# eromero-vlc/superbblas

Measured on AMD Instinct MI355X. Metric: lattice contraction GFLOP/s + permute GB/s, 16^4 spin×color, 1/2/4/8 GPUs, higher is better.
Workload: dtype complex<f64>

## Files before the change

superbblas_amd/csrc/capi.cpp:

```cpp
#include "plan.h"
#include <atomic>
#include <algorithm>
#include <functional>
#include <memory>
#include <unordered_map>

#include <rccl/rccl.h>

#include <cstdlib>
#include <cstring>
#include <mutex>

namespace sbx {
BsrOp *bsr_create(int nd, int ni, int dtype, const std::vector<std::vector<Range>> &pi,
                  const Coor &dimi, const std::vector<std::vector<Range>> &pd, const Coor &dimd,
                  const Coor &blocki, const Coor &blockd, bool block_im_fast,
                  const std::vector<const int *> &ii, const std::vector<const int *> &jj,
                  const std::vector<const void *> &v, const std::vector<int> &devs, bool reverse_jj,
                  const Comm &comm, const Coor *kroni = nullptr, const Coor *krond = nullptr,
                  const std::vector<const void *> *kronv = nullptr);
void bsr_destroy(BsrOp *op);
void bsr_krylov(const BsrOp &op, const Scalar &alpha, const std::string &oi,
                const std::string &od, const DistTensor &x, const Coor &fromx, const Coor &sizex,
                const Scalar &beta, const DistTensor &y, const Coor &fromy, const Coor &sizey,
// ... 365 lines not shown
        if (live) *live = l;
    });
}

int sbx_tune_set(const char *key, long long value) {
    return guard([&] {
        if (!key) throw Error("tune_set: null key");
        const std::string k(key);
        if (k == "copy.budget") g_copy_tune.budget = (long)value;
        else if (k == "copy.run") g_copy_tune.run = (long)value;
        else if (k == "copy.nt") g_copy_tune.nt = (int)value;
        else if (k == "copy.max_elems") g_copy_tune.max_elems = (long)value;
        else if (k == "copy.pair") g_copy_tune.pair = (int)value;
        else if (k == "copy.order") g_copy_tune.order = (int)value;
        else if (k == "copy.trans") g_copy_tune.trans = (int)value;
        else if (k == "copy.btrans") g_copy_tune.btrans = (int)value;
        else if (k == "gemm.max_bytes") g_gemm_tune.max_bytes = (long)value;
        else if (k == "gemm.loaders") g_gemm_tune.loaders = (int)value;
        else if (k == "gemm.dma_spread") g_gemm_tune.dma_spread = (int)value;
        else if (k == "gemm.dma_nt") g_gemm_tune.dma_nt = (int)value;
        else if (k == "gemm.lean") g_gemm_tune.lean = (int)value;
        else if (k == "gemm.skinny") g_gemm_tune.skinny = (int)value;
        else if (k == "bsr.variant") g_bsr_tune.variant = (int)value;
        else if (k == "bsr.row_max_cols") g_bsr_tune.row_max_cols = (long)value;
        else if (k == "bsr.split_max_cols") g_bsr_tune.split_max_cols = (long)value;
        else if (k == "bsr.split_cw") g_bsr_tune.split_cw = (int)value;
        else if (k == "bsr.split_jb") g_bsr_tune.split_jb = (int)value;
        else if (k == "bsr.split_ilv") g_bsr_tune.split_ilv = (int)value;
        else if (k == "bsr.kron_mfma") g_bsr_tune.kron_mfma = (int)value;
        else if (k == "bsr.kron_mfma_min_cols") g_bsr_tune.kron_mfma_min_cols = (long)value;
        else if (k == "bsr.kron_pack") g_bsr_tune.kron_pack = (int)value;
        else if (k == "bsr.kron_xlds") g_bsr_tune.kron_xlds = (int)value;
        else if (k == "bsr.kron_ylds") g_bsr_tune.kron_ylds = (int)value;
        else if (k == "bsr.kron_spin") g_bsr_tune.kron_spin = (int)value;
        else if (k == "bsr.kron_adj") g_bsr_tune.kron_adj = (int)value;
        else if (k == "bsr.kron_spin_min_cols") g_bsr_tune.kron_spin_min_cols = (long)value;
        else if (k == "bsr.kron_order") g_bsr_tune.kron_order = (int)value;
        else if (k == "bsr.nt") g_bsr_tune.nt = (int)value;
        else if (k == "dense.wave") g_dense_wave = (int)value;
        else if (k == "bsr.blk_pd") g_bsr_tune.blk_pd = (int)value;
        else if (k == "bsr.blk_mfma") g_bsr_tune.blk_mfma = (int)value;
        else if (k == "bsr.blk_min") g_bsr_tune.blk_min = (int)value;
        else if (k == "bsr.mixed") g_bsr_tune.mixed = (int)value;
        else if (k == "bsr.adj_inplace") g_bsr_tune.adj_inplace = (int)value;
        else if (k == "bsr.adj_copy_bytes") throw Error("tune_set: bsr.adj_copy_bytes is read-only");
        else if (k == "bsr.tile") g_bsr_tune.tile = (int)value;
        else if (k == "bsr.tile_min_cols") g_bsr_tune.tile_min_cols = value;
        else if (k == "gemm.m3") g_gemm_tune.m3 = (int)value;
        else if (k == "gemm.splits") g_gemm_tune.splits = (int)value;
        else if (k == "gemm.t48") g_gemm_tune.t48 = (int)value;
        else if (k == "gemm.share_ab") g_gemm_tune.share_ab = (int)value;
        else if (k == "gemm.herm") g_gemm_tune.herm = (int)value;
        else if (k == "gemm.frag") g_gemm_tune.frag = (int)value;
        else if (k == "gemm.dot_wgs") g_gemm_tune.dot_wgs = (int)value;
        else if (k == "gemm.frag_tall") g_gemm_tune.frag_tall = (int)value;
        else if (k == "gemm.frag_pair") g_gemm_tune.frag_pair = (int)value;
        else if (k == "gemm.frag_nt") g_gemm_tune.frag_nt = (int)value;
        else if (k == "gemm.frag_small") g_gemm_tune.frag_small = (int)value;
        else if (k == "gemm.frag_uk") g_gemm_tune.frag_uk = (int)value;
        else if (k == "gemm.frag_waves") g_gemm_tune.frag_waves = (int)value;
        else if (k == "gemm.clock") {
            g_gemm_tune.clock = (int)value;
            unsigned long long v[3];
            gemm_clock_read(current_device(), v, true);
        }
        else if (k == "dist.reduce") g_dist_reduce = (int)value;
// ... 12 lines not shown
}

int sbx_tune_get(const char *key, long long *value) {
    return guard([&] {
        if (!key || !value) throw Error("tune_get: null argument");
        const std::string k(key);
        if (k == "copy.budget") *value = g_copy_tune.budget;
        else if (k == "copy.run") *value = g_copy_tune.run;
        else if (k == "copy.nt") *value = g_copy_tune.nt;
        else if (k == "copy.max_elems") *value = g_copy_tune.max_elems;
        else if (k == "copy.pair") *value = g_copy_tune.pair;
        else if (k == "copy.order") *value = g_copy_tune.order;
        else if (k == "copy.trans") *value = g_copy_tune.trans;
        else if (k == "copy.btrans") *value = g_copy_tune.btrans;
        else if (k == "copy.last_pair") *value = g_copy_tune.last_pair;
        else if (k == "gemm.max_bytes") *value = g_gemm_tune.max_bytes;
        else if (k == "gemm.loaders") *value = g_gemm_tune.loaders;
        else if (k == "gemm.dma_spread") *value = g_gemm_tune.dma_spread;
        else if (k == "gemm.dma_nt") *value = g_gemm_tune.dma_nt;
        else if (k == "gemm.lean") *value = g_gemm_tune.lean;
        else if (k == "gemm.last_lean") *value = g_gemm_tune.last_lean;
        else if (k == "gemm.skinny") *value = g_gemm_tune.skinny;
        else if (k == "bsr.variant") *value = g_bsr_tune.variant;
        else if (k == "bsr.row_max_cols") *value = g_bsr_tune.row_max_cols;
        else if (k == "bsr.split_max_cols") *value = g_bsr_tune.split_max_cols;
        else if (k == "bsr.split_cw") *value = g_bsr_tune.split_cw;
        else if (k == "bsr.split_jb") *value = g_bsr_tune.split_jb;
        else if (k == "bsr.split_ilv") *value = g_bsr_tune.split_ilv;
        else if (k == "bsr.kron_mfma") *value = g_bsr_tune.kron_mfma;
        else if (k == "bsr.kron_mfma_min_cols") *value = g_bsr_tune.kron_mfma_min_cols;
        else if (k == "bsr.kron_pack") *value = g_bsr_tune.kron_pack;
        else if (k == "bsr.kron_xlds") *value = g_bsr_tune.kron_xlds;
        else if (k == "bsr.kron_ylds") *value = g_bsr_tune.kron_ylds;
        else if (k == "bsr.kron_spin") *value = g_bsr_tune.kron_spin;
        else if (k == "bsr.kron_adj") *value = g_bsr_tune.kron_adj;
        else if (k == "bsr.kron_spin_min_cols") *value = g_bsr_tune.kron_spin_min_cols;
        else if (k == "bsr.kron_order") *value = g_bsr_tune.kron_order;
        else if (k == "bsr.nt") *value = g_bsr_tune.nt;
        else if (k == "dense.wave") *value = g_dense_wave;
        else if (k == "bsr.blk_pd") *value = g_bsr_tune.blk_pd;
        else if (k == "bsr.blk_mfma") *value = g_bsr_tune.blk_mfma;
        else if (k == "bsr.blk_min") *value = g_bsr_tune.blk_min;
        else if (k == "bsr.tile") *value = g_bsr_tune.tile;
        else if (k == "bsr.tile_min_cols") *value = g_bsr_tune.tile_min_cols;
        else if (k == "bsr.mixed") *value = g_bsr_tune.mixed;
        else if (k == "bsr.last_kernel") *value = g_bsr_tune.last;
        else if (k == "bsr.last_mixed") *value = g_bsr_tune.last_mixed;
        else if (k == "bsr.adj_inplace") *value = g_bsr_tune.adj_inplace;
        else if (k == "bsr.adj_copy_bytes") *value = g_bsr_tune.adj_copy_bytes;
        else if (k == "gemm.m3") *value = g_gemm_tune.m3;
        else if (k == "gemm.splits") *value = g_gemm_tune.splits;
        else if (k == "gemm.t48") *value = g_gemm_tune.t48;
        else if (k == "gemm.share_ab") *value = g_gemm_tune.share_ab;
        else if (k == "gemm.herm") *value = g_gemm_tune.herm;
        else if (k == "gemm.last_herm") *value = g_gemm_tune.last_herm;
        else if (k == "gemm.frag") *value = g_gemm_tune.frag;
        else if (k == "gemm.dot_wgs") *value = g_gemm_tune.dot_wgs;
        else if (k == "gemm.frag_tall") *value = g_gemm_tune.frag_tall;
        else if (k == "gemm.frag_pair") *value = g_gemm_tune.frag_pair;
        else if (k == "gemm.frag_nt") *value = g_gemm_tune.frag_nt;
        else if (k == "gemm.frag_small") *value = g_gemm_tune.frag_small;
        else if (k == "gemm.frag_uk") *value = g_gemm_tune.frag_uk;
        else if (k == "gemm.frag_waves") *value = g_gemm_tune.frag_waves;
        else if (k == "gemm.clock") *value = g_gemm_tune.clock;
        else if (k == "gemm.clock_cycles" || k == "gemm.clock_ticks" || k == "gemm.clock_launches") {
            unsigned long long v[3];
// ... 1058 lines not shown
```

superbblas_amd/csrc/kernels_bsr.hip:

```cpp
#include "elem_ops.h"
#include "sbx_internal.h"

#include <algorithm>
#include <type_traits>

namespace sbx {
BsrTune g_bsr_tune;
namespace {

struct BsrArgs {
    long block_rows;
    int bi, bd;
    const int *ii;
    const int *jj;
    const void *v;
    int block_im_fast;
    const void *x;
    long ldx;
    long x_rows;
    void *y;
    long ldy;
    long ncols;
    double alpha_re, alpha_im;
    int add;
// ... 1501 lines not shown
    }
}

template <typename E>
void gather_typed(const void *src, const int *perm, long nblocks, long be, bool cj, void *dst,
                  hipStream_t s) {
    const long blocks = std::min((nblocks * be + 255) / 256, 65536L);
    hipLaunchKernelGGL(gather_blocks_kernel<E>, dim3((unsigned)blocks), dim3(256), 0, s,
                       (const E *)src, perm, nblocks, be, cj ? 1 : 0, (E *)dst);
    SBX_HIP_CHECK(hipGetLastError());
}

}

void launch_gather_blocks(int t, const void *src, const int *perm, long nblocks, long block_elems,
                          bool conj_values, void *dst, int device) {
    if (nblocks == 0 || block_elems == 0) return;
    set_device(device);
    hipStream_t s = get_stream(device);
    switch (t) {
    case SBX_CDOUBLE: return gather_typed<double2>(src, perm, nblocks, block_elems, conj_values, dst, s);
    case SBX_CFLOAT: return gather_typed<float2>(src, perm, nblocks, block_elems, conj_values, dst, s);
    case SBX_DOUBLE: return gather_typed<double>(src, perm, nblocks, block_elems, false, dst, s);
    case SBX_FLOAT: return gather_typed<float>(src, perm, nblocks, block_elems, false, dst, s);
    case SBX_CHALF: return gather_typed<f16x2>(src, perm, nblocks, block_elems, conj_values, dst, s);
    case SBX_HALF: return gather_typed<f16>(src, perm, nblocks, block_elems, false, dst, s);
    default: throw Error("bsr: unsupported type");
    }
}

void launch_bsr(const BsrDesc &d, int device) {
    if (d.block_rows == 0 || d.ncols == 0) return;
    g_bsr_tune.last = 0;
    set_device(device);
    hipStream_t s = get_stream(device);
    BsrArgs a{};
    a.block_rows = d.block_rows;
    a.bi = d.bi;
    a.bd = d.bd;
    a.ii = d.ii;
    a.jj = d.jj;
    a.v = d.v;
    a.block_im_fast = d.block_im_fast ? 1 : 0;
    a.x = d.x;
    a.ldx = d.ldx;
    a.x_rows = d.x_rows;
    a.y = d.y;
    a.ldy = d.ldy;
    a.ncols = d.ncols;
    a.alpha_re = d.alpha.re;
    a.alpha_im = d.alpha.im;
    a.add = d.add ? 1 : 0;
    a.ilv = 2;
    a.nt = g_bsr_tune.nt;
    a.tiles[0] = d.tiles[0];
    a.tiles[1] = d.tiles[1];
    if (d.adj_ent) {
        const bool yr = d.y_row_major, xr = d.x_row_major;
        if (d.tv == SBX_CFLOAT && d.t == SBX_CDOUBLE) return launch_adj<float2, double2>(a, d.adj_ent, yr, xr, s);
        if (d.tv == SBX_FLOAT && d.t == SBX_DOUBLE) return launch_adj<float, double>(a, d.adj_ent, yr, xr, s);
        if (d.tv == SBX_CHALF && d.t == SBX_CFLOAT) return launch_adj<f16x2, float2>(a, d.adj_ent, yr, xr, s);
        if (d.tv == SBX_HALF && d.t == SBX_FLOAT) return launch_adj<f16, float>(a, d.adj_ent, yr, xr, s);
        if (d.tv != d.t) throw Error("bsr: unsupported pair of value and vector types");
        switch (d.t) {
        case SBX_CDOUBLE: return launch_adj<double2, double2>(a, d.adj_ent, yr, xr, s);
        case SBX_CFLOAT: return launch_adj<float2, float2>(a, d.adj_ent, yr, xr, s);
// ... 27 lines not shown
```

superbblas_amd/csrc/kernels_bsr_kron.hip:

```cpp
#include "elem_ops.h"
#include "sbx_internal.h"

#include <algorithm>
#include <type_traits>

namespace sbx {
namespace {

struct KronArgs {
    long block_rows;
    int nnz;
    int bi, bd, ki, kd;
    const int *jj;
    const void *v;
    const void *kron;
    int block_im_fast;
    const void *x;
    void *y;
    long ncols;
    double alpha_re, alpha_im;
    int add;
    int ylds;
    long x_rows;
    const int *perm;
// ... 196 lines not shown
    const E *__restrict__ x = (const E *)p.x;
    E *__restrict__ y = (E *)p.y;
    const long total = p.block_rows * p.bi * p.ncols * p.ki;
    for (long idx = blockIdx.x * 256L + threadIdx.x; idx < total; idx += (long)gridDim.x * 256L) {
        const int a = (int)(idx % p.ki);
        long t = idx / p.ki;
        const long c = t % p.ncols;
        t /= p.ncols;
        const int i = (int)(t % p.bi);
        const long r = t / p.bi;
        E acc = Ops<E>::zero();
        for (int mu = 0; mu < p.nnz; ++mu) {
            const long j = r * p.nnz + mu;
            const E *xs = x + (long)p.jj[j] * p.bd * p.ncols * p.kd + c * p.kd;
            const E *K = kron + (long)mu * p.ki * p.kd;
            const E *U = v + j * p.bi * p.bd;
            for (int b = 0; b < p.kd; ++b) {
                const E k = p.block_im_fast ? K[a + b * p.ki] : K[a * p.kd + b];
                if (!Ops<E>::nonzero(k)) continue;
                E s = Ops<E>::zero();
                for (int d = 0; d < p.bd; ++d) {
                    const E u = p.block_im_fast ? U[i + d * p.bi] : U[i * p.bd + d];
                    s = Ops<E>::fma(u, xs[d * p.ncols * p.kd + b], s);
                }
                acc = Ops<E>::fma(k, s, acc);
            }
        }
        E o = Ops<E>::scale(acc, p.alpha_re, p.alpha_im);
        if (p.add) o = Ops<E>::add(o, y[idx]);
        y[idx] = o;
    }
}

template <int NNZ, bool kpf = false, int XL = 0>
__global__ void __launch_bounds__(256) bsr_kron_mfma_kernel(const KronArgs p, int ngroups) {
    typedef double2 E;
    const E *__restrict__ x = (const E *)p.x;
    E *__restrict__ y = (E *)p.y;
    const int lane = threadIdx.x & 63;
    const int w = __builtin_amdgcn_readfirstlane(threadIdx.x >> 6);
    const long nchunk = (p.block_rows + 3) / 4;
    const int bid = blockIdx.x, nwg = gridDim.x;
    const int xcd = bid & 7, q8 = nwg >> 3, r8 = nwg & 7;
    const int cnt = xcd < r8 ? q8 + 1 : q8, qx = bid >> 3, npart = cnt / 2;
    const int loc = (npart > 0 && qx < npart * 2) ? (qx % 2) * npart + qx / 2 : qx;
    const long wgi = (xcd < r8 ? xcd * (q8 + 1) : r8 * (q8 + 1) + (xcd - r8) * q8) + loc;
    const long task = wgi * 4 + w;
    const long r = task / ngroups;
    const int cg = (int)(task - r * ngroups);
    __shared__ __attribute__((aligned(16))) E us[(4 * NNZ * 9 + 255) / 256 * 256];
    static_assert(sizeof(us) / sizeof(E) >= (4 * NNZ * 9 + 255) / 256 * 256, "LDS sizing");
    __shared__ __attribute__((aligned(16))) E ks[XL ? NNZ * 16 : 1];
    if constexpr (XL > 0)
        for (int e = (int)threadIdx.x; e < NNZ * 16; e += 256) ks[e] = ((const E *)p.kron)[e];
    {
        const long rlo = (wgi * 4) / ngroups, rhi = min((wgi * 4 + 3) / ngroups, p.block_rows - 1);
        const int nu = (int)(rhi - rlo + 1) * NNZ * 9;
        const __amdgpu_buffer_rsrc_t rs = __builtin_amdgcn_make_buffer_rsrc(
            (void *)p.v, (short)0, (int)(p.block_rows * NNZ * 9 * 16), 0x00020000);
        const unsigned base = (unsigned)(size_t)(const __attribute__((address_space(3))) void *)us +
                              (unsigned)w * 1024u;
        for (int u = 0; u * 256 < nu; ++u) {
            const int e = u * 256 + (int)threadIdx.x;
            const unsigned off = e < nu ? (unsigned)(rlo * NNZ * 9 + e) * 16u : 0x80000000u;
            asm volatile("s_mov_b32 m0, %1\n\t"
                         "s_nop 0\n\t"
                         "buffer_load_dwordx4 %0, %2, 0 offen lds"
                         :
// ... 17 lines not shown
    const int kidx = p.block_im_fast ? ka + kk * 4 : ka * 4 + kk;
    const ConstPtr<int> jrow = (ConstPtr<int>)(p.jj + r * NNZ);
    const long xsite = 3 * n * 4;
    auto load_x = [&](int J, E *xv) {
        const E *xs = x + (long)J * xsite + colc * 4 + b;
#pragma unroll
        for (int d = 0; d < 3; ++d) xv[d] = xs[d * n * 4];
    };
    double accR[3] = {0, 0, 0}, accI[3] = {0, 0, 0};
    E xa[3], xb[3];
    constexpr int NS = XL + 1;
    __shared__ __attribute__((aligned(16))) E xr[XL ? 4 * NS * 3 * 64 : 1];
    const __amdgpu_buffer_rsrc_t rx = __builtin_amdgcn_make_buffer_rsrc((void *)x, (short)0, 0x7fffffff, 0x00020000);
    const int qd = lane >> 2, bd = ((lane & 3) - (qd >> 1) - (qd >> 3)) & 3;
    const long cold = min((long)cg * 16 + qd, n - 1);
    const unsigned xoff_d = (unsigned)(cold * 4 + bd) * 16u;
    const unsigned ring = (unsigned)(size_t)(const __attribute__((address_space(3))) void *)xr + (unsigned)w * (NS * 3072u);
    auto issue_x = [&](int mu) {
        const unsigned base = ring + (unsigned)(mu % NS) * 3072u;
        const unsigned o = (unsigned)((long)jrow[mu] * xsite) * 16u + xoff_d;
#pragma unroll
        for (int d = 0; d < 3; ++d)
            asm volatile("s_mov_b32 m0, %1\n\t"
                         "s_nop 0\n\t"
                         "buffer_load_dwordx4 %0, %2, 0 offen lds"
                         :
                         : "v"(o + (unsigned)(d * n * 4) * 16u),
                           "s"(__builtin_amdgcn_readfirstlane(base + (unsigned)d * 1024u)), "s"(rx)
                         : "memory", "m0");
    };
    const int xpos = 4 * q + ((b + (q >> 1) + (q >> 3)) & 3);
    if constexpr (XL > 0) {
#pragma unroll
        for (int mu = 0; mu < XL && mu < NNZ; ++mu) issue_x(mu);
    } else {
        load_x(jrow[0], xa);
    }
    E Kc = XL > 0 ? E{} : kron[kidx];
#pragma unroll
    for (int mu = 0; mu < NNZ; ++mu) {
        if constexpr (kpf) asm volatile("" ::: "memory");
        E Kn = Kc;
        if constexpr (XL > 0) {
            asm volatile("s_waitcnt lgkmcnt(0)" ::: "memory");
            if (mu + XL < NNZ) issue_x(mu + XL);
            wait_vmcnt(3 * (NNZ - 1 - mu < XL ? NNZ - 1 - mu : XL));
            const E *xs = xr + w * (NS * 192) + (mu % NS) * 192;
#pragma unroll
            for (int d = 0; d < 3; ++d) xa[d] = xs[d * 64 + xpos];
        } else if (mu + 1 < NNZ) {
            load_x(jrow[mu + 1], xb);
            if constexpr (kpf) Kn = kron[(mu + 1) * 16 + kidx];
        }
        const E K = XL > 0 ? ks[mu * 16 + kidx] : kpf ? Kc : kron[mu * 16 + kidx];
        Kc = Kn;
        E t[3];
#pragma unroll
        for (int i = 0; i < 3; ++i) {
            t[i] = Ops<E>::zero();
#pragma unroll
            for (int d = 0; d < 3; ++d) {
                const long ui = mu * 9 + (p.block_im_fast ? i + d * 3 : i * 3 + d);
                t[i] = Ops<E>::fma(urow_s[ui], xa[d], t[i]);
            }
        }
#pragma unroll
        for (int i = 0; i < 3; ++i) {
            accR[i] = __builtin_amdgcn_mfma_f64_4x4x4f64(K.x, t[i].x, accR[i], 0, 0, 0);
            accR[i] = __builtin_amdgcn_mfma_f64_4x4x4f64(-K.y, t[i].y, accR[i], 0, 0, 0);
            accI[i] = __builtin_amdgcn_mfma_f64_4x4x4f64(K.x, t[i].y, accI[i], 0, 0, 0);
            accI[i] = __builtin_amdgcn_mfma_f64_4x4x4f64(K.y, t[i].x, accI[i], 0, 0, 0);
        }
        if (XL == 0 && mu + 1 < NNZ) {
// ... 1 lines not shown
            for (int d = 0; d < 3; ++d) xa[d] = xb[d];
        }
    }
    if constexpr (XL > 0) {
        if (p.ylds) {
            E *ys = xr + w * (NS * 192);
#pragma unroll
            for (int i = 0; i < 3; ++i)
                ys[i * 64 + xpos] = Ops<E>::scale(E{accR[i], accI[i]}, p.alpha_re, p.alpha_im);
            asm volatile("" ::: "memory");
            const long cs = (long)cg * 16 + qd;
            if (cs >= n) return;
            const int ad = bd;
#pragma unroll
            for (int i = 0; i < 3; ++i) {
                E *yp = y + ((r * 3 + i) * n + cs) * 4 + ad;
                E o = ys[i * 64 + lane];
                if (p.add) o = Ops<E>::add(o, *yp);
                *yp = o;
            }
            return;
        }
    }
    if (!ok) return;
#pragma unroll
    for (int i = 0; i < 3; ++i) {
        E *yp = y + ((r * 3 + i) * n + col) * 4 + b;
        E o = Ops<E>::scale(E{accR[i], accI[i]}, p.alpha_re, p.alpha_im);
        if (p.add) o = Ops<E>::add(o, *yp);
        *yp = o;
    }
}

template <int NNZ, bool kpf = false, int XL = 0>
__global__ void __launch_bounds__(256) bsr_kron_mfma_packed_kernel(const KronArgs p, int rw, int xring) {
    constexpr int NS = XL + 1;
    typedef double2 E;
    const E *__restrict__ x = (const E *)p.x;
    E *__restrict__ y = (E *)p.y;
    const int lane = threadIdx.x & 63;
    const int w = __builtin_amdgcn_readfirstlane(threadIdx.x >> 6);
    const int bid = blockIdx.x, nwg = gridDim.x;
    const int xcd = bid & 7, q8 = nwg >> 3, r8 = nwg & 7;
    const int cnt = xcd < r8 ? q8 + 1 : q8, qx = bid >> 3, npart = cnt / 2;
    const int loc = (npart > 0 && qx < npart * 2) ? (qx % 2) * npart + qx / 2 : qx;
    const long wgi = (xcd < r8 ? xcd * (q8 + 1) : r8 * (q8 + 1) + (xcd - r8) * q8) + loc;
    const long r0 = wgi * rw;
    const int nrows = (int)min((long)rw, p.block_rows - r0);
    const long n = p.ncols;
    const int b = lane >> 4, q = lane & 15;
    const int slot = w * 16 + q, rl = slot / (int)n;
    const long col = slot - (long)rl * n;
    const bool live = rl < nrows;
    const int rlc = live ? rl : nrows - 1;
    const long r = r0 + rlc;
    extern __shared__ __attribute__((aligned(16))) char smem_k[];
    E *us = (E *)smem_k;
    {
        const int nu = nrows * NNZ * 9;
        const __amdgpu_buffer_rsrc_t rs = __builtin_amdgcn_make_buffer_rsrc(
            (void *)p.v, (short)0, (int)(p.block_rows * NNZ * 9 * 16), 0x00020000);
        const unsigned base = (unsigned)(size_t)(const __attribute__((address_space(3))) void *)smem_k +
                              (unsigned)w * 1024u;
        const int nth = (int)blockDim.x;
        for (int u = 0; u * nth < nu; ++u) {
            const int e = u * nth + (int)threadIdx.x;
            const unsigned off = e < nu ? (unsigned)(r0 * NNZ * 9 + e) * 16u : 0x80000000u;
            asm volatile("s_mov_b32 m0, %1\n\t"
// ... 8 lines not shown
    int jrow[NNZ];
#pragma unroll
    for (int mu = 0; mu < NNZ; ++mu) jrow[mu] = p.jj[r * NNZ + mu];
    const int ka = lane & 3, kk = lane >> 4;
    const E *kron = (const E *)p.kron;
    const int kidx = p.block_im_fast ? ka + kk * 4 : ka * 4 + kk;
    const long xsite = 3 * n * 4;
    auto load_x = [&](int J, E *xv) {
        const E *xs = x + (long)J * xsite + col * 4 + b;
#pragma unroll
        for (int d = 0; d < 3; ++d) xv[d] = xs[d * n * 4];
    };
    E xa[3], xb[3];
    int jd[XL > 0 ? NNZ : 1];
    unsigned xoff_d = 0, xring_w = 0;
    const __amdgpu_buffer_rsrc_t rx = __builtin_amdgcn_make_buffer_rsrc((void *)x, (short)0, 0x7fffffff, 0x00020000);
    if constexpr (XL > 0) {
        const int qd = lane >> 2, bd = ((lane & 3) - (qd >> 1) - (qd >> 3)) & 3;
        const int sd = w * 16 + qd, rld = sd / (int)n;
        const long cold = sd - (long)rld * n;
        const long rd = r0 + (rld < nrows ? rld : nrows - 1);
#pragma unroll
        for (int mu = 0; mu < NNZ; ++mu) jd[mu] = p.jj[rd * NNZ + mu];
        xoff_d = (unsigned)(cold * 4 + bd) * 16u;
        xring_w = (unsigned)xring + (unsigned)w * (NS * 3072u);
    }
    const unsigned lds0 = (unsigned)(size_t)(const __attribute__((address_space(3))) void *)smem_k;
    E *ks = (E *)(smem_k + xring + (int)(blockDim.x >> 6) * NS * 3072);
    if constexpr (XL > 0) {
        for (int e = (int)threadIdx.x; e < NNZ * 16; e += (int)blockDim.x) ks[e] = kron[e];
#pragma unroll
        for (int mu = 0; mu < NNZ; ++mu) asm volatile("" : "+v"(jd[mu]));
    }
    auto issue_x = [&](int mu) {
        const unsigned base = lds0 + xring_w + (unsigned)(mu % NS) * 3072u;
        const unsigned o = (unsigned)((long)jd[mu] * xsite) * 16u + xoff_d;
#pragma unroll
        for (int d = 0; d < 3; ++d)
            asm volatile("s_mov_b32 m0, %1\n\t"
                         "s_nop 0\n\t"
                         "buffer_load_dwordx4 %0, %2, 0 offen lds"
                         :
                         : "v"(o + (unsigned)(d * n * 4) * 16u),
                           "s"(__builtin_amdgcn_readfirstlane(base + (unsigned)d * 1024u)), "s"(rx)
                         : "memory", "m0");
    };
    const int xpos = 4 * q + ((b + (q >> 1) + (q >> 3)) & 3);
    if constexpr (XL > 0) {
#pragma unroll
        for (int mu = 0; mu < XL && mu < NNZ; ++mu) issue_x(mu);
    } else {
        load_x(jrow[0], xa);
    }
    asm volatile("s_waitcnt vmcnt(0)" ::: "memory");
    __syncthreads();
    const E *urow_s = us + rlc * NNZ * 9;
    double accR[3] = {0, 0, 0}, accI[3] = {0, 0, 0};
    E Kc = XL > 0 ? E{} : kron[kidx];
#pragma unroll
    for (int mu = 0; mu < NNZ; ++mu) {
        if constexpr (kpf) asm volatile("" ::: "memory");
        E Kn = Kc;
        if constexpr (XL > 0) {
            asm volatile("s_waitcnt lgkmcnt(0)" ::: "memory");
            if (mu + XL < NNZ) issue_x(mu + XL);
            wait_vmcnt(3 * (NNZ - 1 - mu < XL ? NNZ - 1 - mu : XL));
            const E *xs = (const E *)(smem_k + xring_w + (mu % NS) * 3072);
#pragma unroll
            for (int d = 0; d < 3; ++d) xa[d] = xs[d * 64 + xpos];
        } else if (mu + 1 < NNZ) {
            load_x(jrow[mu + 1], xb);
            if constexpr (kpf) Kn = kron[(mu + 1) * 16 + kidx];
        }
        const E K = XL > 0 ? ks[mu * 16 + kidx] : kpf ? Kc : kron[mu * 16 + kidx];
        Kc = Kn;
        E t[3];
#pragma unroll
        for (int i = 0; i < 3; ++i) {
            t[i] = Ops<E>::zero();
#pragma unroll
            for (int d = 0; d < 3; ++d) {
                const long ui = mu * 9 + (p.block_im_fast ? i + d * 3 : i * 3 + d);
                t[i] = Ops<E>::fma(urow_s[ui], xa[d], t[i]);
            }
        }
#pragma unroll
        for (int i = 0; i < 3; ++i) {
            accR[i] = __builtin_amdgcn_mfma_f64_4x4x4f64(K.x, t[i].x, accR[i], 0, 0, 0);
            accR[i] = __builtin_amdgcn_mfma_f64_4x4x4f64(-K.y, t[i].y, accR[i], 0, 0, 0);
            accI[i] = __builtin_amdgcn_mfma_f64_4x4x4f64(K.x, t[i].y, accI[i], 0, 0, 0);
            accI[i] = __builtin_amdgcn_mfma_f64_4x4x4f64(K.y, t[i].x, accI[i], 0, 0, 0);
        }
        if (XL == 0 && mu + 1 < NNZ) {
#pragma unroll
            for (int d = 0; d < 3; ++d) xa[d] = xb[d];
        }
    }
    if constexpr (XL > 0) {
        if (p.ylds) {
            E *ys = (E *)(smem_k + xring_w);
#pragma unroll
            for (int i = 0; i < 3; ++i)
                ys[i * 64 + xpos] = Ops<E>::scale(E{accR[i], accI[i]}, p.alpha_re, p.alpha_im);
            asm volatile("" ::: "memory");
            const int qd = lane >> 2, ad = ((lane & 3) - (qd >> 1) - (qd >> 3)) & 3;
            const int sd = w * 16 + qd, rld = sd / (int)n;
            if (rld >= nrows) return;
            const long cold = sd - (long)rld * n;
#pragma unroll
            for (int i = 0; i < 3; ++i) {
                E *yp = y + (((r0 + rld) * 3 + i) * n + cold) * 4 + ad;
                E o = ys[i * 64 + lane];
                if (p.add) o = Ops<E>::add(o, *yp);
                *yp = o;
            }
            return;
        }
    }
    if (!live) return;
#pragma unroll
    for (int i = 0; i < 3; ++i) {
        E *yp = y + ((r * 3 + i) * n + col) * 4 + b;
        E o = Ops<E>::scale(E{accR[i], accI[i]}, p.alpha_re, p.alpha_im);
        if (p.add) o = Ops<E>::add(o, *yp);
        *yp = o;
    }
}


constexpr int KS_WAVE_LDS = 2 * 4096 + 2 * 512 + 2 * 256;

__device__ __forceinline__ void dma16(unsigned off, unsigned base, __amdgpu_buffer_rsrc_t r) {
    asm volatile("s_mov_b32 m0, %1\n\t"
                 "s_nop 0\n\t"
                 "buffer_load_dwordx4 %0, %2, 0 offen lds"
                 :
                 : "v"(off), "s"(__builtin_amdgcn_readfirstlane(base)), "s"(r)
                 : "memory", "m0");
}
__device__ __forceinline__ void dma4(unsigned off, unsigned base, __amdgpu_buffer_rsrc_t r) {
    asm volatile("s_mov_b32 m0, %1\n\t"
                 "s_nop 0\n\t"
                 "buffer_load_dword %0, %2, 0 offen lds"
                 :
                 : "v"(off), "s"(__builtin_amdgcn_readfirstlane(base)), "s"(r)
                 : "memory", "m0");
}

__global__ void __launch_bounds__(256) bsr_kron_spin_kernel(const KronArgs p) {
    typedef double2 E;
// ... 425 lines not shown
template <typename E> void launch_kron_adj_typed(const KronAdjArgs &a, hipStream_t s) {
    KernelTimer timer("bsr", s);
    if (g_bsr_tune.kron_adj && a.bi == 3 && a.bd == 3 && a.ki == 4 && a.kd == 4) {
        const int cpg = (int)std::min<long>(a.ncols, 256);
        const bool stage = a.ncols >= KRON_ADJ_STAGE_COLS && g_bsr_tune.kron_adj != 2;
        const int S = std::min(256 / cpg, stage ? KRON_ADJ_SITES : 256);
        const int nth = (S * cpg + 63) / 64 * 64;
        const long gx = (a.sites + S - 1) / S, gy = (a.ncols + cpg - 1) / cpg;
        const long lds = (long)((stage ? KRON_ADJ_CHUNK * 9 : 0) + (long)a.nnz * 16) * (long)sizeof(E);
        if (lds <= KRON_LDS_BYTES && gx < (1L << 31) && gy < 65536) {
            g_bsr_tune.last = 15;
            if (stage)
                hipLaunchKernelGGL((bsr_kron_adj_kernel<E, 3, 3, 4, 4, true>), dim3((unsigned)gx, (unsigned)gy),
                                   dim3(nth), (size_t)lds, s, a, S, cpg);
            else
                hipLaunchKernelGGL((bsr_kron_adj_kernel<E, 3, 3, 4, 4, false>), dim3((unsigned)gx, (unsigned)gy),
                                   dim3(nth), (size_t)lds, s, a, S, cpg);
            SBX_HIP_CHECK(hipGetLastError());
            return;
        }
    }
    g_bsr_tune.last = 16;
    const long total = a.sites * a.bd * a.ncols * a.kd;
    const long blocks = std::min((total + 255) / 256, 65536L);
    hipLaunchKernelGGL((bsr_kron_adj_generic_kernel<E>), dim3(blocks), dim3(256), 0, s, a);
    SBX_HIP_CHECK(hipGetLastError());
}

void launch_bsr_kron_adj(const BsrDesc &d, int device) {
    if (d.num_nnz_per_row <= 0 || !d.kron || !d.adj_ent || !d.x_row_major || !d.y_row_major)
        throw Error("kron bsr: internal error (adjoint layout or pattern)");
    set_device(device);
    g_bsr_tune.last = 0;
    KronAdjArgs a{};
    a.sites = d.block_rows;
    a.nnz = d.num_nnz_per_row;
    a.bi = d.bd;
    a.bd = d.bi;
    a.ki = d.kd;
    a.kd = d.ki;
    a.ptr = d.adj_ptr;
    a.ent = d.adj_ent;
    a.v = d.v;
    a.kron = d.kron;
    a.block_im_fast = d.block_im_fast ? 0 : 1;
    a.x = d.x;
    a.y = d.y;
    a.ncols = d.ncols;
    a.alpha_re = d.alpha.re;
    a.alpha_im = d.alpha.im;
    a.add = d.add ? 1 : 0;
    hipStream_t s = get_stream(device);
    switch (d.t) {
    case SBX_CDOUBLE: return launch_kron_adj_typed<double2>(a, s);
    case SBX_CFLOAT: return launch_kron_adj_typed<float2>(a, s);
    case SBX_DOUBLE: return launch_kron_adj_typed<double>(a, s);
    case SBX_FLOAT: return launch_kron_adj_typed<float>(a, s);
    default: throw Error("kron bsr: unsupported type");
    }
}

template <typename E> void launch_kron_typed(const KronArgs &a, hipStream_t s) {
    KernelTimer timer("bsr", s);
    const long row_bytes = (long)a.nnz * (a.bi * a.bd * sizeof(E) + sizeof(int));
    if constexpr (std::is_same<E, double2>::value) {
        if (g_bsr_tune.kron_spin == 2 && a.xtab && a.bi == 3 && a.bd == 3 && a.ki == 4 && a.kd == 4 &&
// ... 15 lines not shown
            a.block_rows * a.ncols + 1024 < (1L << 31)) {
            const long waves = (a.block_rows * a.ncols + 63) / 64, blocks = (waves + 3) / 4;
            if (blocks < (1L << 31)) {
                g_bsr_tune.last = 9;
                const size_t lds = 4 * (size_t)KS_WAVE_LDS;
                hipLaunchKernelGGL(bsr_kron_spin_kernel, dim3((unsigned)blocks), dim3(256), lds, s, a);
                SBX_HIP_CHECK(hipGetLastError());
                return;
            }
        }
        if (g_bsr_tune.kron_mfma && a.bi == 3 && a.bd == 3 && a.ki == 4 && a.kd == 4 && a.nnz == 9 &&
            a.ncols >= g_bsr_tune.kron_mfma_min_cols && a.block_rows * 81L * 16 < (1L << 31)) {
            int wpk = 0;
            for (int wv = 4; wv >= 1 && g_bsr_tune.kron_pack; --wv)
                if (a.ncols < 16 && (16 * wv) % a.ncols == 0 && 16 * wv / a.ncols <= 32) {
                    wpk = wv;
                    break;
                }
            if (wpk > 0) {
                const int rw = (int)(16 * wpk / a.ncols);
                const long blocks = (a.block_rows + rw - 1) / rw;
                if (blocks < (1L << 31)) {
                    g_bsr_tune.last = 6;
                    const int nth = 64 * wpk;
                    const size_t lds_cb = (size_t)((rw * 81 + nth - 1) / nth * nth) * 16;
                    check_dma_lds("bsr_kron_mfma_packed_kernel", lds_cb, (rw * 81L + nth - 1) / nth, nth);
                    const int xl = std::max(a.block_rows * 12L, a.x_rows * 4L) * a.ncols * 16 < (1L << 31)
                                       ? std::max(0, std::min(3, g_bsr_tune.kron_xlds)) : 0;
                    const size_t lds_bytes = lds_cb + (xl > 0 ? (size_t)wpk * (xl + 1) * 3072 + 9 * 16 * 16 : 0);
                    if (xl) check_dma_lds("bsr_kron_mfma_packed_kernel x ring", lds_bytes, 0, 0, (long)lds_cb + wpk * (xl + 1) * 3072L + 9 * 16 * 16);
                    auto go = [&](auto kern) {
                        hipLaunchKernelGGL(kern, dim3((unsigned)blocks), dim3(64 * wpk), lds_bytes, s, a, rw, (int)lds_cb);
                    };
                    if (xl == 1) go(bsr_kron_mfma_packed_kernel<9, true, 1>);
                    else if (xl == 2) go(bsr_kron_mfma_packed_kernel<9, true, 2>);
                    else if (xl == 3) go(bsr_kron_mfma_packed_kernel<9, true, 3>);
                    else
                        hipLaunchKernelGGL((bsr_kron_mfma_packed_kernel<9, true>), dim3((unsigned)blocks),
                                           dim3(64 * wpk), lds_bytes, s, a, rw, (int)lds_cb);
                    SBX_HIP_CHECK(hipGetLastError());
                    return;
                }
            }
            const long ngroups = (a.ncols + 15) / 16;
            const long tasks = a.block_rows * ngroups, blocks = (tasks + 3) / 4;
            if (blocks < (1L << 31)) {
                g_bsr_tune.last = 5;
                const int xl = std::max(a.block_rows * 12L, a.x_rows * 4L) * a.ncols * 16 < (1L << 31)
                                   ? std::max(0, std::min(3, g_bsr_tune.kron_xlds)) : 0;
                auto go = [&](auto kern) {
                    hipLaunchKernelGGL(kern, dim3((unsigned)blocks), dim3(256), 0, s, a, (int)ngroups);
                };
                if (xl == 1) go(bsr_kron_mfma_kernel<9, false, 1>);
                else if (xl == 2) go(bsr_kron_mfma_kernel<9, false, 2>);
                else if (xl == 3) go(bsr_kron_mfma_kernel<9, false, 3>);
                else
                    hipLaunchKernelGGL((bsr_kron_mfma_kernel<9, false>), dim3((unsigned)blocks), dim3(256), 0,
                                       s, a, (int)ngroups);
                SBX_HIP_CHECK(hipGetLastError());
                return;
            }
        }
    }
    if (a.bi == 3 && a.bd == 3 && a.ki == 4 && a.kd == 4 && a.nnz == 9 && a.ncols >= 4 &&
        row_bytes * (256 / std::min<long>(a.ncols, 256)) <= KRON_LDS_BYTES) {
        const int cpg = (int)std::min<long>(a.ncols, 256);
        const int S = 256 / cpg;
        const dim3 grid((unsigned)((a.block_rows + S - 1) / S), (unsigned)((a.ncols + cpg - 1) / cpg));
        hipLaunchKernelGGL((bsr_kron_lds_kernel<E, 3, 3, 4, 4, 9>), grid, dim3(256),
                           (size_t)(row_bytes * S), s, a, S, cpg);
    } else if (a.bi == 3 && a.bd == 3 && a.ki == 4 && a.kd == 4) {
        const long total = a.block_rows * a.ncols;
        const long blocks = std::min((total + 255) / 256, 65536L);
        hipLaunchKernelGGL((bsr_kron_kernel<E, 3, 3, 4, 4>), dim3(blocks), dim3(256), 0, s, a);
    } else {
        const long total = a.block_rows * a.bi * a.ncols * a.ki;
        const long blocks = std::min((total + 255) / 256, 65536L);
        hipLaunchKernelGGL((bsr_kron_generic_kernel<E>), dim3(blocks), dim3(256), 0, s, a);
    }
    SBX_HIP_CHECK(hipGetLastError());
}

}

void launch_bsr_kron(const BsrDesc &d, int device) {
    if (d.block_rows == 0 || d.ncols == 0) return;
    if (d.adj_ptr) return launch_bsr_kron_adj(d, device);
    if (d.num_nnz_per_row <= 0 || !d.kron || !d.x_row_major || !d.y_row_major)
        throw Error("kron bsr: internal error (layout or pattern)");
    set_device(device);
    g_bsr_tune.last = 0;
    hipStream_t s = get_stream(device);
    KronArgs a{};
    a.block_rows = d.block_rows;
    a.nnz = d.num_nnz_per_row;
    a.bi = d.bi;
    a.bd = d.bd;
    a.ki = d.ki;
    a.kd = d.kd;
    a.jj = d.jj;
    a.v = d.v;
    a.kron = d.kron;
    a.block_im_fast = d.block_im_fast ? 1 : 0;
    a.x = d.x;
    a.y = d.y;
    a.ncols = d.ncols;
    a.alpha_re = d.alpha.re;
    a.alpha_im = d.alpha.im;
    a.add = d.add ? 1 : 0;
    a.ylds = g_bsr_tune.kron_ylds ? 1 : 0;
    a.x_rows = d.x_rows > 0 ? d.x_rows : d.block_rows * d.bd;
    a.perm = g_bsr_tune.kron_order ? d.kron_perm : nullptr;
    a.ktab = d.kron_terms;
    a.xtab = d.kron_xor;
    switch (d.t) {
    case SBX_CDOUBLE: return launch_kron_typed<double2>(a, s);
    case SBX_CFLOAT: return launch_kron_typed<float2>(a, s);
    case SBX_DOUBLE: return launch_kron_typed<double>(a, s);
    case SBX_FLOAT: return launch_kron_typed<float>(a, s);
    default: throw Error("kron bsr: unsupported type");
    }
}

}
// ... 1 lines not shown
```

superbblas_amd/csrc/sbx_internal.h:

```cpp
#pragma once

#include <hip/hip_runtime.h>

#include <array>
#include <atomic>
#include <complex>
#include <cstdint>
#include <cstring>
#include <memory>
#include <stdexcept>
#include <string>
#include <vector>

#include "../../include/superbblas_amd/sbx.h"

namespace sbx {

struct Error : public std::runtime_error {
    explicit Error(const std::string &s) : std::runtime_error(s) {}
};

#define SBX_HIP_CHECK(expr)                                                                        \
    do {                                                                                           \
        hipError_t sbx_e_ = (expr);                                                                \
// ... 157 lines not shown
    int herm = 0;
    std::atomic<int> last_herm{0};
    int loaders = 8;
    int dma_spread = 1;
    int dma_nt = 0;
    int lean = 1;
    std::atomic<int> last_lean{0};
    int skinny = 1;
    int clock = 0;
    int dot_wgs = 256;
    int frag_uk = 0;
    int frag_waves = 4096;
    int frag = 1;
    int frag_small = 32;
    int frag_nt = 0;
    int frag_pair = 1;
    int frag_tall = 0;
};
uint32_t storage_checksum(const void *p, std::size_t bytes, std::size_t blocksize, uint32_t prev);
void gemm_clock_read(int device, unsigned long long out[3], bool reset);
extern GemmTune g_gemm_tune;
struct BsrTune {
    int variant = 0;
    long row_max_cols = 3;
    long split_max_cols = 32;
    int split_cw = 0;
    int split_jb = 0;
    int split_ilv = 2;
    int kron_mfma = 1;
    long kron_mfma_min_cols = 8;
    int kron_pack = 1;
    int kron_xlds = 1;
    int kron_ylds = 0;
    int kron_spin = 0;
    long kron_spin_min_cols = 8;
    int kron_order = 1;
    int kron_adj = 1;
    int blk_pd = 1;
    int tile = 0;
    long tile_min_cols = 33;
    int nt = 11;
    int blk_mfma = 1;
    int blk_min = 16;
    int mixed = 1;
    int adj_inplace = 0;
    std::atomic<long long> adj_copy_bytes{0};
    std::atomic<int> last{0};
    std::atomic<int> last_mixed{0};
};
extern BsrTune g_bsr_tune;
extern int g_dense_wave;

inline void check_dma_lds(const char *kernel, size_t lds, long passes, long lanes_per_pass,
                   long extra_bytes = 0) {
    const long need = passes * lanes_per_pass * 16 + extra_bytes;
    if ((long)lds < need)
        throw Error(std::string("bsr: internal LDS sizing error in ") + kernel + ": " +
                    std::to_string(lds) + " bytes for DMA passes needing " + std::to_string(need));
}

void launch_zero(void *p, std::size_t bytes, int device);

struct IndexCopyDesc {
    int src_t, dst_t;
    const void *src;
    void *dst;
    const int *src_idx = nullptr, *dst_idx = nullptr;
    long n = 0, blocking = 1;
    Scalar alpha;
    bool add = false;
};
void launch_index_copy(const IndexCopyDesc &d, int device);

struct TileSched {
    const int *rows = nullptr, *uniq = nullptr;
    const unsigned char *loc = nullptr;
    int umax = 0, tt = 0;
    long chunks = 0;
};

struct BsrDesc {
// ... 45 lines not shown
```

Before: 73890.

## Add lean software-pipelined MFMA path for kron BSR kernels

Adds a lean variant of the kron MFMA kernels, enabled by default, that double-buffers x neighbour loads through buffer-to-LDS DMA two steps ahead. It overlaps the spin-color FMA of the next neighbour with the MFMA accumulation of the previous one, using explicit sched barriers and waitcnt placement. It also pins the occupancy target through waves_per_eu and adds a direct per-lane epilogue for the packed kernel. The aim is to hide load latency and reduce register pressure, at the cost of hand-tuned asm scheduling that may be fragile or spill.

```diff
diff --git a/superbblas_amd/csrc/capi.cpp b/superbblas_amd/csrc/capi.cpp
--- a/superbblas_amd/csrc/capi.cpp
+++ b/superbblas_amd/csrc/capi.cpp
@@ -421,6 +421,7 @@
         else if (k == "bsr.kron_pack") g_bsr_tune.kron_pack = (int)value;
         else if (k == "bsr.kron_xlds") g_bsr_tune.kron_xlds = (int)value;
         else if (k == "bsr.kron_ylds") g_bsr_tune.kron_ylds = (int)value;
+        else if (k == "bsr.kron_lean") g_bsr_tune.kron_lean = (int)value;
         else if (k == "bsr.kron_spin") g_bsr_tune.kron_spin = (int)value;
         else if (k == "bsr.kron_adj") g_bsr_tune.kron_adj = (int)value;
         else if (k == "bsr.kron_spin_min_cols") g_bsr_tune.kron_spin_min_cols = (long)value;
@@ -499,6 +500,8 @@
         else if (k == "bsr.kron_pack") *value = g_bsr_tune.kron_pack;
         else if (k == "bsr.kron_xlds") *value = g_bsr_tune.kron_xlds;
         else if (k == "bsr.kron_ylds") *value = g_bsr_tune.kron_ylds;
+        else if (k == "bsr.kron_lean") *value = g_bsr_tune.kron_lean;
+        else if (k == "bsr.last_kron_lean") *value = g_bsr_tune.last_kron_lean;
         else if (k == "bsr.kron_spin") *value = g_bsr_tune.kron_spin;
         else if (k == "bsr.kron_adj") *value = g_bsr_tune.kron_adj;
         else if (k == "bsr.kron_spin_min_cols") *value = g_bsr_tune.kron_spin_min_cols;
diff --git a/superbblas_amd/csrc/kernels_bsr.hip b/superbblas_amd/csrc/kernels_bsr.hip
--- a/superbblas_amd/csrc/kernels_bsr.hip
+++ b/superbblas_amd/csrc/kernels_bsr.hip
@@ -1557,6 +1557,7 @@
 void launch_bsr(const BsrDesc &d, int device) {
     if (d.block_rows == 0 || d.ncols == 0) return;
     g_bsr_tune.last = 0;
+    g_bsr_tune.last_kron_lean = 0;
     set_device(device);
     hipStream_t s = get_stream(device);
     BsrArgs a{};
diff --git a/superbblas_amd/csrc/kernels_bsr_kron.hip b/superbblas_amd/csrc/kernels_bsr_kron.hip
--- a/superbblas_amd/csrc/kernels_bsr_kron.hip
+++ b/superbblas_amd/csrc/kernels_bsr_kron.hip
@@ -252,8 +252,69 @@
     }
 }
 
-template <int NNZ, bool kpf = false, int XL = 0>
-__global__ void __launch_bounds__(256) bsr_kron_mfma_kernel(const KronArgs p, int ngroups) {
+__device__ __forceinline__ void dma16_so(unsigned voff, unsigned soff, unsigned base, __amdgpu_buffer_rsrc_t r) {
+    asm volatile("s_mov_b32 m0, %1\n\t"
+                 "s_nop 0\n\t"
+                 "buffer_load_dwordx4 %0, %2, %3 offen lds"
+                 :
+                 : "v"(voff), "s"(base), "s"(r), "s"(soff)
+                 : "memory", "m0");
+}
+
+template <int NNZ, bool BIF, bool LATE, typename Issue>
+__device__ __forceinline__ void kron_lean_steps(const double2 *urow_s, const double2 *ring, const double2 *ksl,
+                                                int xpos, Issue issue, double (&accR)[3], double (&accI)[3]) {
+    typedef double2 E;
+    E tp[3] = {}, Kp = {};
+#pragma unroll
+    for (int mu = 0; mu <= NNZ; ++mu) {
+        E xa[3] = {}, u[9] = {};
+        auto read_u = [&](int d) {
+#pragma unroll
+            for (int i = 0; i < 3; ++i) u[i * 3 + d] = urow_s[mu * 9 + (BIF ? d * 3 + i : i * 3 + d)];
+        };
+        if (mu < NNZ) {
+            wait_vmcnt(mu + 1 < NNZ ? 3 : 0);
+            const E *xs = ring + (mu % 2) * 192;
+#pragma unroll
+            for (int d = 0; d < 3; ++d) xa[d] = xs[d * 64 + xpos];
+#pragma unroll
+            for (int d = 0; d < (LATE ? 2 : 3); ++d) read_u(d);
+        }
+        if (mu > 0) {
+#pragma unroll
+            for (int i = 0; i < 3; ++i) {
+                accR[i] = __builtin_amdgcn_mfma_f64_4x4x4f64(Kp.x, tp[i].x, accR[i], 0, 0, 0);
+                accI[i] = __builtin_amdgcn_mfma_f64_4x4x4f64(Kp.x, tp[i].y, accI[i], 0, 0, 0);
+            }
+#pragma unroll
+            for (int i = 0; i < 3; ++i) {
+                accR[i] = __builtin_amdgcn_mfma_f64_4x4x4f64(Kp.y, tp[i].y, accR[i], 0, 0, 1);
+                accI[i] = __builtin_amdgcn_mfma_f64_4x4x4f64(Kp.y, tp[i].x, accI[i], 0, 0, 0);
+            }
+        }
+        if (mu < NNZ) {
+            __builtin_amdgcn_sched_barrier(0);
+            asm volatile("s_waitcnt lgkmcnt(0)" ::: "memory");
+            if (mu + 2 < NNZ) issue(mu + 2);
+            Kp = ksl[mu * 16];
+#pragma unroll
+            for (int d = 0; d < 3; ++d) {
+#pragma unroll
+                for (int i = 0; i < 3; ++i) tp[i] = Ops<E>::fma(u[i * 3 + d], xa[d], d ? tp[i] : Ops<E>::zero());
+                if (LATE && d == 0) {
+                    __builtin_amdgcn_sched_barrier(0);
+                    read_u(2);
+                }
+            }
+            __builtin_amdgcn_sched_barrier(0);
+        }
+    }
+}
+
+template <int NNZ, bool kpf = false, int XL = 0, bool LEAN = false>
+__global__ void __launch_bounds__(256) __attribute__((amdgpu_waves_per_eu(LEAN ? 4 : 1, LEAN ? 5 : 8)))
+bsr_kron_mfma_kernel(const KronArgs p, int ngroups) {
     typedef double2 E;
     const E *__restrict__ x = (const E *)p.x;
     E *__restrict__ y = (E *)p.y;
@@ -337,13 +398,31 @@
     const int xpos = 4 * q + ((b + (q >> 1) + (q >> 3)) & 3);
     if constexpr (XL > 0) {
 #pragma unroll
-        for (int mu = 0; mu < XL && mu < NNZ; ++mu) issue_x(mu);
+        for (int mu = 0; mu < (LEAN ? 2 : XL) && mu < NNZ; ++mu) issue_x(mu);
     } else {
         load_x(jrow[0], xa);
     }
+    if constexpr (LEAN) {
+        static_assert(XL == 1, "the lean steps: x one neighbour ahead");
+        unsigned so[NNZ];
+#pragma unroll
+        for (int mu = 0; mu < NNZ; ++mu) {
+            so[mu] = (unsigned)((long)jrow[mu] * xsite) * 16u;
+            asm volatile("" : "+s"(so[mu]));
+        }
+        const unsigned dstep = (unsigned)(n * 4) * 16u;
+        auto issue = [&](int mu) {
+#pragma unroll
+            for (int d = 0; d < 3; ++d)
+                dma16_so(xoff_d, so[mu] + (unsigned)d * dstep, ring + (unsigned)(mu % 2) * 3072u + (unsigned)d * 1024u, rx);
+        };
+        const E *rg = xr + w * (NS * 192);
+        if (p.block_im_fast) kron_lean_steps<NNZ, true, false>(urow_s, rg, ks + kidx, xpos, issue, accR, accI);
+        else kron_lean_steps<NNZ, false, false>(urow_s, rg, ks + kidx, xpos, issue, accR, accI);
+    }
     E Kc = XL > 0 ? E{} : kron[kidx];
 #pragma unroll
-    for (int mu = 0; mu < NNZ; ++mu) {
+    for (int mu = 0; mu < (LEAN ? 0 : NNZ); ++mu) {
         if constexpr (kpf) asm volatile("" ::: "memory");
         E Kn = Kc;
         if constexpr (XL > 0) {
@@ -411,8 +490,9 @@
     }
 }
 
-template <int NNZ, bool kpf = false, int XL = 0>
-__global__ void __launch_bounds__(256) bsr_kron_mfma_packed_kernel(const KronArgs p, int rw, int xring) {
+template <int NNZ, bool kpf = false, int XL = 0, bool LEAN = false>
+__global__ void __launch_bounds__(256) __attribute__((amdgpu_waves_per_eu(LEAN ? 5 : 1, LEAN ? 5 : 8)))
+bsr_kron_mfma_packed_kernel(const KronArgs p, int rw, int xring) {
     constexpr int NS = XL + 1;
     typedef double2 E;
     const E *__restrict__ x = (const E *)p.x;
@@ -487,6 +567,15 @@
 #pragma unroll
         for (int mu = 0; mu < NNZ; ++mu) asm volatile("" : "+v"(jd[mu]));
     }
+    unsigned xo[LEAN ? NNZ : 1];
+    if constexpr (LEAN) {
+        static_assert(XL == 1, "the lean steps: x one neighbour ahead");
+#pragma unroll
+        for (int mu = 0; mu < NNZ; ++mu) {
+            xo[mu] = (unsigned)((long)jd[mu] * xsite) * 16u + xoff_d;
+            asm volatile("" : "+v"(xo[mu]));
+        }
+    }
     auto issue_x = [&](int mu) {
         const unsigned base = lds0 + xring_w + (unsigned)(mu % NS) * 3072u;
         const unsigned o = (unsigned)((long)jd[mu] * xsite) * 16u + xoff_d;
@@ -503,7 +592,7 @@
     const int xpos = 4 * q + ((b + (q >> 1) + (q >> 3)) & 3);
     if constexpr (XL > 0) {
 #pragma unroll
-        for (int mu = 0; mu < XL && mu < NNZ; ++mu) issue_x(mu);
+        for (int mu = 0; mu < (LEAN ? 2 : XL) && mu < NNZ; ++mu) issue_x(mu);
     } else {
         load_x(jrow[0], xa);
     }
@@ -511,9 +600,20 @@
     __syncthreads();
     const E *urow_s = us + rlc * NNZ * 9;
     double accR[3] = {0, 0, 0}, accI[3] = {0, 0, 0};
+    if constexpr (LEAN) {
+        const unsigned dstep = (unsigned)(n * 4) * 16u;
+        auto issue = [&](int mu) {
+#pragma unroll
+            for (int d = 0; d < 3; ++d)
+                dma16_so(xo[mu], (unsigned)d * dstep, lds0 + xring_w + (unsigned)(mu % 2) * 3072u + (unsigned)d * 1024u, rx);
+        };
+        const E *rg = (const E *)(smem_k + xring_w);
+        if (p.block_im_fast) kron_lean_steps<NNZ, true, true>(urow_s, rg, ks + kidx, xpos, issue, accR, accI);
+        else kron_lean_steps<NNZ, false, true>(urow_s, rg, ks + kidx, xpos, issue, accR, accI);
+    }
     E Kc = XL > 0 ? E{} : kron[kidx];
 #pragma unroll
-    for (int mu = 0; mu < NNZ; ++mu) {
+    for (int mu = 0; mu < (LEAN ? 0 : NNZ); ++mu) {
         if constexpr (kpf) asm volatile("" ::: "memory");
         E Kn = Kc;
         if constexpr (XL > 0) {
@@ -571,6 +671,21 @@
             }
             return;
         }
+    }
+    if constexpr (LEAN) {
+        int le = lane;
+        asm volatile("" : "+v"(le));
+        const int sle = w * 16 + (le & 15), rle = sle / (int)n;
+        if (rle >= nrows) return;
+        const long re = r0 + rle, cole = sle - (long)rle * n;
+#pragma unroll
+        for (int i = 0; i < 3; ++i) {
+            E *yp = y + ((re * 3 + i) * n + cole) * 4 + (le >> 4);
+            E o = Ops<E>::scale(E{accR[i], accI[i]}, p.alpha_re, p.alpha_im);
+            if (p.add) o = Ops<E>::add(o, *yp);
+            *yp = o;
+        }
+        return;
     }
     if (!live) return;
 #pragma unroll
@@ -1062,6 +1177,7 @@
         throw Error("kron bsr: internal error (adjoint layout or pattern)");
     set_device(device);
     g_bsr_tune.last = 0;
+    g_bsr_tune.last_kron_lean = 0;
     KronAdjArgs a{};
     a.sites = d.block_rows;
     a.nnz = d.num_nnz_per_row;
@@ -1143,7 +1259,10 @@
                     auto go = [&](auto kern) {
                         hipLaunchKernelGGL(kern, dim3((unsigned)blocks), dim3(64 * wpk), lds_bytes, s, a, rw, (int)lds_cb);
                     };
-                    if (xl == 1) go(bsr_kron_mfma_packed_kernel<9, true, 1>);
+                    const bool lean = g_bsr_tune.kron_lean && xl == 1 && !a.ylds && g_bsr_tune.kron_spin == 0;
+                    g_bsr_tune.last_kron_lean = lean ? 1 : 0;
+                    if (lean) go(bsr_kron_mfma_packed_kernel<9, true, 1, true>);
+                    else if (xl == 1) go(bsr_kron_mfma_packed_kernel<9, true, 1>);
                     else if (xl == 2) go(bsr_kron_mfma_packed_kernel<9, true, 2>);
                     else if (xl == 3) go(bsr_kron_mfma_packed_kernel<9, true, 3>);
                     else
@@ -1162,7 +1281,10 @@
                 auto go = [&](auto kern) {
                     hipLaunchKernelGGL(kern, dim3((unsigned)blocks), dim3(256), 0, s, a, (int)ngroups);
                 };
-                if (xl == 1) go(bsr_kron_mfma_kernel<9, false, 1>);
+                const bool lean = g_bsr_tune.kron_lean && xl == 1 && !a.ylds && g_bsr_tune.kron_spin == 0;
+                g_bsr_tune.last_kron_lean = lean ? 1 : 0;
+                if (lean) go(bsr_kron_mfma_kernel<9, false, 1, true>);
+                else if (xl == 1) go(bsr_kron_mfma_kernel<9, false, 1>);
                 else if (xl == 2) go(bsr_kron_mfma_kernel<9, false, 2>);
                 else if (xl == 3) go(bsr_kron_mfma_kernel<9, false, 3>);
                 else
@@ -1201,6 +1323,7 @@
         throw Error("kron bsr: internal error (layout or pattern)");
     set_device(device);
     g_bsr_tune.last = 0;
+    g_bsr_tune.last_kron_lean = 0;
     hipStream_t s = get_stream(device);
     KronArgs a{};
     a.block_rows = d.block_rows;
diff --git a/superbblas_amd/csrc/sbx_internal.h b/superbblas_amd/csrc/sbx_internal.h
--- a/superbblas_amd/csrc/sbx_internal.h
+++ b/superbblas_amd/csrc/sbx_internal.h
@@ -213,6 +213,7 @@
     int kron_pack = 1;
     int kron_xlds = 1;
     int kron_ylds = 0;
+    int kron_lean = 1;
     int kron_spin = 0;
     long kron_spin_min_cols = 8;
     int kron_order = 1;
@@ -228,6 +229,7 @@
     std::atomic<long long> adj_copy_bytes{0};
     std::atomic<int> last{0};
     std::atomic<int> last_mixed{0};
+    std::atomic<int> last_kron_lean{0};
 };
 extern BsrTune g_bsr_tune;
 extern int g_dense_wave;
```

New measurement: 74110 (median of 5 runs). Within noise of the previous version (+0.3%).
